# dhansmair/flamingo-mini

Measured on AMD Instinct MI355X. Metric: images/sec (fwd+bwd) flamingo-mini bs=32, higher is better.
Workload: dtype bf16

## Files before the change

flamingo-mini_amd/csrc/ff_optim.hip:

```cpp
#include <algorithm>
#include <cstdlib>
#include <type_traits>
#include "ff_common.h"
#include "ff_internal.h"

namespace ff {

constexpr int kAdamTensors = 32;
constexpr int kAdamChunk = 256 * 128;

struct AdamTable {
    void* p[kAdamTensors];
    const void* g[kAdamTensors];
    void* m[kAdamTensors];
    void* v[kAdamTensors];
    float* w[kAdamTensors];
    long long n[kAdamTensors];
    int block_start[kAdamTensors + 1];
    int count;
    float lr, beta1, beta2, eps, decay, bc1, bc2_sqrt, grad_scale;
    const float* step_dev;
    const float* lr_dev;
    const float* grad_coef;
};

template <typename T, typename ST, bool MASTER, int VEC, int MODE = 0, bool CLIP = false, typename GT = T>
__global__ __launch_bounds__(256) void adamw_kernel(const AdamTable t) {
    int ti = 0;
#pragma unroll 1
    while (ti + 1 < t.count && (int)blockIdx.x >= t.block_start[ti + 1]) ti++;
    const long long n = t.n[ti];
    const long long base = (long long)((int)blockIdx.x - t.block_start[ti]) * kAdamChunk;
    T* p = (T*)t.p[ti];
    const GT* g = (const GT*)t.g[ti];
    ST* m = (ST*)t.m[ti];
    ST* v = (ST*)t.v[ti];
    float* w = t.w[ti];
    float bc1 = t.bc1, bc2_sqrt = t.bc2_sqrt;
    if (t.step_dev) {
        const float step = *t.step_dev;
        bc1 = 1.f - powf(t.beta1, step);
        bc2_sqrt = sqrtf(1.f - powf(t.beta2, step));
    }
    const float lr = t.lr_dev ? *t.lr_dev : t.lr;
    float clip_scale = 0.f;
    if constexpr (CLIP) clip_scale = t.grad_scale * *t.grad_coef;
    const float step_size = lr / bc1, keep = 1.f - lr * t.decay;
    bool vec = VEC > 1 && n % VEC == 0 && ((uintptr_t)p | (uintptr_t)g | (uintptr_t)m | (uintptr_t)v) % 16 == 0;
    if (MASTER) vec = vec && (uintptr_t)w % 16 == 0;
    auto ldv = [&](auto* q, long long i, float (&o)[VEC], auto stream) {
        typedef std::remove_cv_t<std::remove_pointer_t<decltype(q)>> Q;
        constexpr int QN = Vec<Q>::N;
#pragma unroll
        for (int c = 0; c < VEC / QN; c++) {
            float part[QN];
            if constexpr (decltype(stream)::value && MODE >= 1) Vec<Q>::load_nt(q + i + c * QN, part);
            else Vec<Q>::load(q + i + c * QN, part);
#pragma unroll
            for (int e = 0; e < QN; e++) o[c * QN + e] = part[e];
        }
    };
    auto stv = [&](auto* q, long long i, const float (&o)[VEC], auto stream) {
        typedef std::remove_pointer_t<decltype(q)> Q;
        constexpr int QN = Vec<Q>::N;
#pragma unroll
        for (int c = 0; c < VEC / QN; c++) {
            float part[QN];
#pragma unroll
            for (int e = 0; e < QN; e++) part[e] = o[c * QN + e];
            if constexpr (decltype(stream)::value && MODE >= 1) Vec<Q>::store_nt(q + i + c * QN, part);
            else Vec<Q>::store(q + i + c * QN, part);
        }
    };
    const long long end = min(n, base + (long long)kAdamChunk);
    auto update = [&](float (&pf)[VEC], const float (&gf)[VEC], float (&mf)[VEC], float (&vf)[VEC]) {
#pragma unroll
        for (int e = 0; e < VEC; e++) {
            float gr;
            if constexpr (CLIP) gr = gf[e] * clip_scale;
            else gr = gf[e] * t.grad_scale;
            pf[e] *= keep;
            mf[e] = t.beta1 * mf[e] + (1.f - t.beta1) * gr;
            vf[e] = t.beta2 * vf[e] + (1.f - t.beta2) * gr * gr;
            pf[e] -= step_size * mf[e] / (sqrtf(vf[e]) / bc2_sqrt + t.eps);
        }
    };
    if (vec) {
        constexpr std::true_type S{};
        constexpr std::false_type K{};
        auto store = [&](long long i, const float (&pf)[VEC], const float (&mf)[VEC], const float (&vf)[VEC]) {
            stv(p, i, pf, K); stv(m, i, mf, S); stv(v, i, vf, S);
            if (MASTER) stv(w, i, pf, S);
        };
        long long i = base + (long long)threadIdx.x * VEC;
        for (; i + 256 * VEC < end; i += 512 * VEC) {
            const long long j = i + 256 * VEC;
            float p0[VEC], g0[VEC], m0[VEC], v0[VEC], p1[VEC], g1[VEC], m1[VEC], v1[VEC];
            if (MASTER) { ldv(w, i, p0, S); ldv(w, j, p1, S); } else { ldv(p, i, p0, K); ldv(p, j, p1, K); }
            ldv(g, i, g0, S); ldv(g, j, g1, S);
            ldv(m, i, m0, S); ldv(m, j, m1, S);
            ldv(v, i, v0, S); ldv(v, j, v1, S);
            update(p0, g0, m0, v0);
            update(p1, g1, m1, v1);
            store(i, p0, m0, v0);
            store(j, p1, m1, v1);
        }
        if (i < end) {
            float pf[VEC], gf[VEC], mf[VEC], vf[VEC];
            if (MASTER) ldv(w, i, pf, S); else ldv(p, i, pf, K);
            ldv(g, i, gf, S); ldv(m, i, mf, S); ldv(v, i, vf, S);
            update(pf, gf, mf, vf);
            store(i, pf, mf, vf);
        }
        return;
    }
    for (long long i = base + (long long)threadIdx.x * VEC; i < end; i += 256 * VEC) {
        float pf[VEC], gf[VEC], mf[VEC], vf[VEC];
#pragma unroll
        for (int e = 0; e < VEC; e++) {
            const bool ok = i + e < n;
            pf[e] = ok ? (MASTER ? w[i + e] : to_f32(p[i + e])) : 0.f; gf[e] = ok ? to_f32(g[i + e]) : 0.f;
            mf[e] = ok ? to_f32(m[i + e]) : 0.f; vf[e] = ok ? to_f32(v[i + e]) : 0.f;
        }
        update(pf, gf, mf, vf);
#pragma unroll
        for (int e = 0; e < VEC; e++)
            if (i + e < n) {
                p[i + e] = from_f32<T>(pf[e]); m[i + e] = from_f32<ST>(mf[e]); v[i + e] = from_f32<ST>(vf[e]);
                if (MASTER) w[i + e] = pf[e];
            }
    }
}

template <bool CLIP>
static void adamw_dispatch(int dtype, bool master, int state_dtype, dim3 grid, hipStream_t stream, const AdamTable& t) {
    const dim3 block(256);
    if (dtype == FF_DTYPE_F32) adamw_kernel<float, float, false, 4, 0, CLIP><<<grid, block, 0, stream>>>(t);
    else if (master) adamw_kernel<bf16, float, true, 8, 1, CLIP><<<grid, block, 0, stream>>>(t);
    else if (state_dtype == FF_DTYPE_F32) adamw_kernel<bf16, float, false, 8, 1, CLIP><<<grid, block, 0, stream>>>(t);
    else {
        static const int mode = CLIP ? 1 : dbg_switch("FF_ADAMW_MODE", 1);
        if (mode >= 1) adamw_kernel<bf16, bf16, false, 8, 1, CLIP><<<grid, block, 0, stream>>>(t);
        else if constexpr (!CLIP) adamw_kernel<bf16, bf16, false, 8><<<grid, block, 0, stream>>>(t);
    }
}

template <bool CLIP>
static void adamw_dispatch_acc(bool master, int state_dtype, dim3 grid, hipStream_t stream, const AdamTable& t) {
    const dim3 block(256);
    if (master) adamw_kernel<bf16, float, true, 8, 1, CLIP, float><<<grid, block, 0, stream>>>(t);
    else if (state_dtype == FF_DTYPE_F32) adamw_kernel<bf16, float, false, 8, 1, CLIP, float><<<grid, block, 0, stream>>>(t);
    else adamw_kernel<bf16, bf16, false, 8, 1, CLIP, float><<<grid, block, 0, stream>>>(t);
}

static int adamw_launch(const ff_adamw_desc* d, int state_dtype, void* const* params, const void* const* grads, void* const* exp_avg,
                        void* const* exp_avg_sq, float* const* master, const float* lr_dev, const float* grad_coef, const long long* numels,
                        hipStream_t stream, bool acc_grads = false) {
    FF_CHECK(d && params && grads && exp_avg && exp_avg_sq && numels, FF_ERR_SHAPE, "ff_adamw_step: null argument");
    FF_CHECK(d->dtype == FF_DTYPE_F32 || d->dtype == FF_DTYPE_BF16, FF_ERR_UNSUPPORTED, "ff_adamw_step: dtype %d", d->dtype);
    FF_CHECK(state_dtype == d->dtype || state_dtype == FF_DTYPE_F32, FF_ERR_UNSUPPORTED, "ff_adamw_step: moments must be stored in the parameter dtype or in fp32");
    FF_CHECK(!master || d->dtype == FF_DTYPE_BF16, FF_ERR_UNSUPPORTED, "ff_adamw_step: fp32 master copies go with bf16 parameters");
    FF_CHECK(d->n_tensors >= 0 && (d->step >= 1 || d->step_dev), FF_ERR_SHAPE, "ff_adamw_step: n_tensors=%d step=%d", d->n_tensors, d->step);
    AdamTable t;
    t.lr = d->lr; t.beta1 = d->beta1; t.beta2 = d->beta2; t.eps = d->eps; t.decay = d->weight_decay;
    t.step_dev = d->step_dev;
    t.lr_dev = lr_dev;
    t.grad_coef = grad_coef;
    t.bc1 = 1.f - powf(d->beta1, (float)std::max(d->step, 1));
    t.bc2_sqrt = sqrtf(1.f - powf(d->beta2, (float)std::max(d->step, 1)));
    t.grad_scale = d->grad_scale == 0.f ? 1.f : d->grad_scale;
    int i = 0;
    while (i < d->n_tensors) {
        int cnt = 0, blocks = 0;
        while (i < d->n_tensors && cnt < kAdamTensors) {
            if (numels[i] > 0) {
                FF_CHECK(params[i] && grads[i] && exp_avg[i] && exp_avg_sq[i] && (!master || master[i]), FF_ERR_SHAPE, "ff_adamw_step: tensor %d has a null pointer", i);
                t.p[cnt] = params[i]; t.g[cnt] = grads[i]; t.m[cnt] = exp_avg[i]; t.v[cnt] = exp_avg_sq[i]; t.n[cnt] = numels[i];
                t.w[cnt] = master ? master[i] : nullptr;
                t.block_start[cnt] = blocks;
                blocks += cdiv(numels[i], kAdamChunk);
                cnt++;
            }
            i++;
        }
        if (!cnt) break;
        t.block_start[cnt] = blocks;
        t.count = cnt;
        const dim3 grid(blocks);
        if (master) FF_CHECK(state_dtype == FF_DTYPE_F32, FF_ERR_UNSUPPORTED, "ff_adamw_step: fp32 master copies go with fp32 moments");
        if (acc_grads && d->dtype == FF_DTYPE_BF16) {
            if (grad_coef) adamw_dispatch_acc<true>(master != nullptr, state_dtype, grid, stream, t);
            else adamw_dispatch_acc<false>(master != nullptr, state_dtype, grid, stream, t);
        } else if (grad_coef) adamw_dispatch<true>(d->dtype, master != nullptr, state_dtype, grid, stream, t);
        else adamw_dispatch<false>(d->dtype, master != nullptr, state_dtype, grid, stream, t);
        FF_TRY(check_launch("adamw"));
    }
    return FF_OK;
}


struct GradTable {
    void* g[kAdamTensors];
    long long n[kAdamTensors];
    int block_start[kAdamTensors + 1];
    int count;
    float scale;
    float* partials;
    const float* coef;
};
constexpr long long kGradMaxBlocks = 1 << 22;

template <typename T>
__global__ __launch_bounds__(256) void grad_sumsq_kernel(const GradTable t) {
    __shared__ float red[4];
    constexpr int VEC = Vec<T>::N, PIECES = 8;
    int ti = 0;
#pragma unroll 1
    while (ti + 1 < t.count && (int)blockIdx.x >= t.block_start[ti + 1]) ti++;
    const long long n = t.n[ti];
    const long long base = (long long)((int)blockIdx.x - t.block_start[ti]) * kAdamChunk;
    const long long end = min(n, base + (long long)kAdamChunk);
    const T* g = (const T*)t.g[ti];
    const float scale = t.scale;
    float acc = 0.f;
    long long tail = base;
    if ((uintptr_t)g % 16 == 0) {
        const long long vend = base + (end - base) / VEC * VEC;
        tail = vend;
        long long i = base + (long long)threadIdx.x * VEC;
        for (; i + (PIECES - 1) * 256 * VEC < vend; i += PIECES * 256 * VEC) {
            typename Vec<T>::raw r[PIECES];
#pragma unroll
            for (int k = 0; k < PIECES; k++) r[k] = __builtin_nontemporal_load((const typename Vec<T>::raw*)(g + i + k * 256 * VEC));
#pragma unroll
            for (int k = 0; k < PIECES; k++)
#pragma unroll
                for (int e = 0; e < VEC; e++) {
                    const float x = (float)r[k][e] * scale;
                    acc = fmaf(x, x, acc);
                }
        }
        for (; i < vend; i += 256 * VEC) {
            float x[VEC];
            Vec<T>::load_nt(g + i, x);
#pragma unroll
            for (int e = 0; e < VEC; e++) {
                const float y = x[e] * scale;
                acc = fmaf(y, y, acc);
            }
        }
    }
    for (long long i = tail + threadIdx.x; i < end; i += 256) {
        const float x = to_f32(g[i]) * scale;
        acc = fmaf(x, x, acc);
    }
    acc = block_sum<4>(acc, red);
    if (threadIdx.x == 0) t.partials[blockIdx.x] = acc;
}

__global__ __launch_bounds__(1024) void grad_sumsq_reduce_kernel(const float* partials, long long n, double* sum, int accumulate) {
    __shared__ double red[16];
    double s = 0.0;
    long long i = threadIdx.x;
    for (; i + 3 * 1024 < n; i += 4 * 1024) {
        const float a = partials[i], b = partials[i + 1024], c = partials[i + 2048], d = partials[i + 3072];
        s += (double)a; s += (double)b; s += (double)c; s += (double)d;
    }
    for (; i < n; i += 1024) s += (double)partials[i];
#pragma unroll
    for (int o = 32; o > 0; o >>= 1) s += __shfl_xor(s, o, 64);
    if ((threadIdx.x & 63) == 0) red[threadIdx.x >> 6] = s;
    __syncthreads();
    if (threadIdx.x == 0) {
        double total = accumulate ? *sum : 0.0;
        for (int w = 0; w < 16; w++) total += red[w];
        *sum = total;
    }
}

__global__ void grad_clip_coef_kernel(const double* sum, float max_norm, float* norm, float* coef) {
    if (threadIdx.x != 0) return;
    const float nrm = (float)sqrt(*sum);
    const float c = max_norm / (nrm + 1e-6f);
    if (norm) *norm = nrm;
    if (coef) *coef = c > 1.f ? 1.f : c;
}

template <typename T>
__global__ __launch_bounds__(256) void grad_scale_kernel(const GradTable t) {
    constexpr int VEC = Vec<T>::N;
    int ti = 0;
#pragma unroll 1
    while (ti + 1 < t.count && (int)blockIdx.x >= t.block_start[ti + 1]) ti++;
    const long long n = t.n[ti];
    const long long base = (long long)((int)blockIdx.x - t.block_start[ti]) * kAdamChunk;
    const long long end = min(n, base + (long long)kAdamChunk);
    T* g = (T*)t.g[ti];
    const float c = *t.coef;
    long long tail = base;
    if ((uintptr_t)g % 16 == 0) {
        const long long vend = base + (end - base) / VEC * VEC;
        tail = vend;
        for (long long i = base + (long long)threadIdx.x * VEC; i < vend; i += 256 * VEC) {
            float x[VEC];
            Vec<T>::load(g + i, x);
#pragma unroll
            for (int e = 0; e < VEC; e++) x[e] *= c;
            Vec<T>::store(g + i, x);
        }
    }
    for (long long i = tail + threadIdx.x; i < end; i += 256) g[i] = from_f32<T>(to_f32(g[i]) * c);
}

struct AccTable {
    const void* g[kAdamTensors];
    float* a[kAdamTensors];
    long long n[kAdamTensors];
    int block_start[kAdamTensors + 1];
    int count;
    float scale;
};

template <typename T, bool OVERWRITE>
__global__ __launch_bounds__(256) void grad_accumulate_kernel(const AccTable t) {
    constexpr int VEC = Vec<T>::N, PIECES = 4;
    int ti = 0;
#pragma unroll 1
    while (ti + 1 < t.count && (int)blockIdx.x >= t.block_start[ti + 1]) ti++;
    const long long n = t.n[ti];
    const long long base = (long long)((int)blockIdx.x - t.block_start[ti]) * kAdamChunk;
    const long long end = min(n, base + (long long)kAdamChunk);
    const T* g = (const T*)t.g[ti];
    float* a = t.a[ti];
    const float s = t.scale;
    auto lda = [&](long long i, float (&o)[VEC]) {
#pragma unroll
        for (int c = 0; c < VEC / 4; c++) {
            float part[4];
            Vec<float>::load_nt(a + i + c * 4, part);
#pragma unroll
            for (int e = 0; e < 4; e++) o[c * 4 + e] = part[e];
        }
    };
    auto sta = [&](long long i, const float (&o)[VEC]) {
#pragma unroll
        for (int c = 0; c < VEC / 4; c++) {
            float part[4];
#pragma unroll
            for (int e = 0; e < 4; e++) part[e] = o[c * 4 + e];
            Vec<float>::store_nt(a + i + c * 4, part);
        }
    };
    auto fold = [&](float gf, float af) { return OVERWRITE ? s * gf : fmaf(s, gf, af); };
    long long tail = base;
    if (((uintptr_t)g | (uintptr_t)a) % 16 == 0) {
        const long long vend = base + (end - base) / VEC * VEC;
        tail = vend;
        long long i = base + (long long)threadIdx.x * VEC;
        for (; i + (PIECES - 1) * 256 * VEC < vend; i += PIECES * 256 * VEC) {
            float gf[PIECES][VEC], af[PIECES][VEC];
#pragma unroll
            for (int k = 0; k < PIECES; k++) Vec<T>::load_nt(g + i + k * 256 * VEC, gf[k]);
            if constexpr (!OVERWRITE) {
#pragma unroll
                for (int k = 0; k < PIECES; k++) lda(i + k * 256 * VEC, af[k]);
            }
#pragma unroll
            for (int k = 0; k < PIECES; k++) {
#pragma unroll
                for (int e = 0; e < VEC; e++) af[k][e] = fold(gf[k][e], OVERWRITE ? 0.f : af[k][e]);
                sta(i + k * 256 * VEC, af[k]);
            }
        }
        for (; i < vend; i += 256 * VEC) {
            float gf[VEC], af[VEC];
            Vec<T>::load_nt(g + i, gf);
            if constexpr (!OVERWRITE) lda(i, af);
#pragma unroll
            for (int e = 0; e < VEC; e++) af[e] = fold(gf[e], OVERWRITE ? 0.f : af[e]);
            sta(i, af);
        }
    }
    for (long long i = tail + threadIdx.x; i < end; i += 256)
        a[i] = fold(to_f32(g[i]), OVERWRITE ? 0.f : a[i]);
}

static long long grad_slots(int n_tensors, const long long* numels) {
    long long slots = 0;
    for (int i = 0; i < n_tensors; i++)
        if (numels[i] > 0) slots += (numels[i] + kAdamChunk - 1) / kAdamChunk;
    return slots;
}

template <typename F>
static int grad_launches(const char* what, int n_tensors, void* const* grads, const long long* numels, GradTable& t, F&& launch) {
    FF_CHECK(n_tensors >= 0 && (n_tensors == 0 || (grads && numels)), FF_ERR_SHAPE, "%s: null argument", what);
    long long slot = 0;
    int i = 0;
    while (i < n_tensors) {
        int cnt = 0;
        long long blocks = 0;
        while (i < n_tensors && cnt < kAdamTensors) {
            if (numels[i] > 0) {
                const long long b = (numels[i] + kAdamChunk - 1) / kAdamChunk;
                FF_CHECK(b <= kGradMaxBlocks, FF_ERR_SHAPE, "%s: tensor %d has %lld elements", what, i, numels[i]);
                if (blocks + b > kGradMaxBlocks) break;
                FF_CHECK(grads[i], FF_ERR_SHAPE, "%s: tensor %d has a null pointer", what, i);
                t.g[cnt] = grads[i]; t.n[cnt] = numels[i];
                t.block_start[cnt] = (int)blocks;
                blocks += b;
                cnt++;
            }
            i++;
        }
        if (!cnt) break;
        t.block_start[cnt] = (int)blocks;
        t.count = cnt;
        launch(t, (int)blocks, slot);
        FF_TRY(check_launch(what));
        slot += blocks;
    }
    return FF_OK;
}

}

extern "C" int ff_adamw_step(const ff_adamw_desc* d, void* const* params, const void* const* grads, void* const* exp_avg,
                             void* const* exp_avg_sq, const long long* numels, ff_stream_t stream) {
    return ff::adamw_launch(d, d ? d->dtype : 0, params, grads, exp_avg, exp_avg_sq, nullptr, nullptr, nullptr, numels, (hipStream_t)stream);
}
extern "C" int ff_adamw_step_mixed(const ff_adamw_desc* d, int state_dtype, void* const* params, const void* const* grads, void* const* exp_avg,
                                   void* const* exp_avg_sq, float* const* master, const float* lr_dev, const long long* numels,
                                   ff_stream_t stream) {
    return ff::adamw_launch(d, state_dtype, params, grads, exp_avg, exp_avg_sq, master, lr_dev, nullptr, numels, (hipStream_t)stream);
}

extern "C" int ff_adamw_step_clipped(const ff_adamw_desc* d, int state_dtype, void* const* params, const void* const* grads, void* const* exp_avg,
                                     void* const* exp_avg_sq, float* const* master, const float* lr_dev, const float* grad_coef,
                                     const long long* numels, ff_stream_t stream) {
    FF_CHECK(grad_coef, FF_ERR_SHAPE, "ff_adamw_step_clipped: grad_coef is null");
    return ff::adamw_launch(d, state_dtype, params, grads, exp_avg, exp_avg_sq, master, lr_dev, grad_coef, numels, (hipStream_t)stream);
}
extern "C" int ff_adamw_step_acc(const ff_adamw_desc* d, int state_dtype, void* const* params, const float* const* grads32, void* const* exp_avg,
                                 void* const* exp_avg_sq, float* const* master, const float* lr_dev, const float* grad_coef,
                                 const long long* numels, ff_stream_t stream) {
    return ff::adamw_launch(d, state_dtype, params, (const void* const*)grads32, exp_avg, exp_avg_sq, master, lr_dev, grad_coef, numels,
                            (hipStream_t)stream, true);
}
extern "C" long long ff_grad_sumsq_partials(int n_tensors, const long long* numels) {
    return n_tensors > 0 && numels ? ff::grad_slots(n_tensors, numels) : 0;
}
extern "C" int ff_grad_sumsq(int dtype, int n_tensors, const void* const* grads, const long long* numels, float scale, float* partials,
                             long long n_partials, ff_stream_t stream) {
    using namespace ff;
    FF_CHECK(dtype == FF_DTYPE_F32 || dtype == FF_DTYPE_BF16, FF_ERR_UNSUPPORTED, "ff_grad_sumsq: dtype %d", dtype);
    FF_CHECK(n_tensors >= 0 && (n_tensors == 0 || numels), FF_ERR_SHAPE, "ff_grad_sumsq: null argument");
    const long long need = n_tensors > 0 ? grad_slots(n_tensors, numels) : 0;
    FF_CHECK(need <= n_partials && (need == 0 || partials), FF_ERR_WORKSPACE, "ff_grad_sumsq: %lld partials needed, %lld given", need, n_partials);
    GradTable t;
    t.scale = scale;
    t.coef = nullptr;
    return grad_launches("ff_grad_sumsq", n_tensors, (void* const*)grads, numels, t, [&](GradTable& tt, int blocks, long long slot) {
        tt.partials = partials + slot;
        if (dtype == FF_DTYPE_F32) grad_sumsq_kernel<float><<<blocks, 256, 0, (hipStream_t)stream>>>(tt);
        else grad_sumsq_kernel<bf16><<<blocks, 256, 0, (hipStream_t)stream>>>(tt);
    });
}
extern "C" int ff_grad_sumsq_reduce(const float* partials, long long n_partials, double* sum, int accumulate, ff_stream_t stream) {
    FF_CHECK(sum && n_partials >= 0 && (n_partials == 0 || partials), FF_ERR_SHAPE, "ff_grad_sumsq_reduce: null argument");
    ff::grad_sumsq_reduce_kernel<<<1, 1024, 0, (hipStream_t)stream>>>(partials, n_partials, sum, accumulate);
    return ff::check_launch("ff_grad_sumsq_reduce");
}
extern "C" int ff_grad_clip_coef(const double* sum, float max_norm, float* norm, float* coef, ff_stream_t stream) {
    FF_CHECK(sum && (norm || coef), FF_ERR_SHAPE, "ff_grad_clip_coef: null argument");
    ff::grad_clip_coef_kernel<<<1, 64, 0, (hipStream_t)stream>>>(sum, max_norm, norm, coef);
    return ff::check_launch("ff_grad_clip_coef");
}
extern "C" int ff_scale_grads(int dtype, int n_tensors, void* const* grads, const long long* numels, const float* coef, ff_stream_t stream) {
    using namespace ff;
    FF_CHECK(dtype == FF_DTYPE_F32 || dtype == FF_DTYPE_BF16, FF_ERR_UNSUPPORTED, "ff_scale_grads: dtype %d", dtype);
    FF_CHECK(coef, FF_ERR_SHAPE, "ff_scale_grads: coef is null");
    GradTable t;
    t.scale = 1.f;
    t.partials = nullptr;
    t.coef = coef;
    return grad_launches("ff_scale_grads", n_tensors, grads, numels, t, [&](GradTable& tt, int blocks, long long) {
        if (dtype == FF_DTYPE_F32) grad_scale_kernel<float><<<blocks, 256, 0, (hipStream_t)stream>>>(tt);
        else grad_scale_kernel<bf16><<<blocks, 256, 0, (hipStream_t)stream>>>(tt);
    });
}
extern "C" int ff_grad_accumulate(int dtype, int n_tensors, const void* const* grads, float* const* acc, const long long* numels, float scale,
                                  int overwrite, ff_stream_t stream) {
    using namespace ff;
    const char* what = "ff_grad_accumulate";
    FF_CHECK(dtype == FF_DTYPE_F32 || dtype == FF_DTYPE_BF16, FF_ERR_UNSUPPORTED, "%s: dtype %d", what, dtype);
    FF_CHECK(n_tensors >= 0 && (n_tensors == 0 || (grads && acc && numels)), FF_ERR_SHAPE, "%s: null argument", what);
    AccTable t;
    t.scale = scale;
    int i = 0;
    while (i < n_tensors) {
        int cnt = 0;
        long long blocks = 0;
        while (i < n_tensors && cnt < kAdamTensors) {
            if (numels[i] > 0) {
                const long long b = (numels[i] + kAdamChunk - 1) / kAdamChunk;
                FF_CHECK(b <= kGradMaxBlocks, FF_ERR_SHAPE, "%s: tensor %d has %lld elements", what, i, numels[i]);
                if (blocks + b > kGradMaxBlocks) break;
                FF_CHECK(grads[i] && acc[i], FF_ERR_SHAPE, "%s: tensor %d has a null pointer", what, i);
                t.g[cnt] = grads[i]; t.a[cnt] = acc[i]; t.n[cnt] = numels[i];
                t.block_start[cnt] = (int)blocks;
                blocks += b;
                cnt++;
            }
            i++;
        }
        if (!cnt) break;
        t.block_start[cnt] = (int)blocks;
        t.count = cnt;
        const dim3 grid((unsigned)blocks);
        hipStream_t s = (hipStream_t)stream;
        if (dtype == FF_DTYPE_F32) {
            if (overwrite) grad_accumulate_kernel<float, true><<<grid, 256, 0, s>>>(t);
            else grad_accumulate_kernel<float, false><<<grid, 256, 0, s>>>(t);
        } else {
            if (overwrite) grad_accumulate_kernel<bf16, true><<<grid, 256, 0, s>>>(t);
            else grad_accumulate_kernel<bf16, false><<<grid, 256, 0, s>>>(t);
        }
        FF_TRY(check_launch(what));
    }
    return FF_OK;
}
```

Before: 790.4.

## Make AdamW kernel persistent with occupancy-sized grid and smaller work items

The AdamW kernel now runs as a persistent grid-stride loop over smaller work items instead of one block per large chunk. Grid size comes from a cached CU count times the kernel's measured occupancy. Per-block setup (bias correction, lr load) is hoisted out of the item loop, and launch bounds add a minimum-waves hint per dtype. This aims to balance load across tensors of uneven size and cut tail effects, at the cost of a serial tensor-index walk per block and possible register pressure from the occupancy hint.

```diff
diff --git a/flamingo-mini_amd/csrc/ff_optim.hip b/flamingo-mini_amd/csrc/ff_optim.hip
--- a/flamingo-mini_amd/csrc/ff_optim.hip
+++ b/flamingo-mini_amd/csrc/ff_optim.hip
@@ -1,4 +1,5 @@
 #include <algorithm>
+#include <atomic>
 #include <cstdlib>
 #include <type_traits>
 #include "ff_common.h"
@@ -8,6 +9,8 @@
 
 constexpr int kAdamTensors = 32;
 constexpr int kAdamChunk = 256 * 128;
+constexpr int kAdamItem = 256 * 16;
+constexpr long long kAdamMaxItems = 1 << 30;
 
 struct AdamTable {
     void* p[kAdamTensors];
@@ -16,7 +19,7 @@
     void* v[kAdamTensors];
     float* w[kAdamTensors];
     long long n[kAdamTensors];
-    int block_start[kAdamTensors + 1];
+    int item_start[kAdamTensors + 1];
     int count;
     float lr, beta1, beta2, eps, decay, bc1, bc2_sqrt, grad_scale;
     const float* step_dev;
@@ -24,28 +27,14 @@
     const float* grad_coef;
 };
 
-template <typename T, typename ST, bool MASTER, int VEC, int MODE = 0, bool CLIP = false, typename GT = T>
-__global__ __launch_bounds__(256) void adamw_kernel(const AdamTable t) {
-    int ti = 0;
-#pragma unroll 1
-    while (ti + 1 < t.count && (int)blockIdx.x >= t.block_start[ti + 1]) ti++;
+template <typename T, typename ST, bool MASTER, int VEC, int MODE, bool CLIP, typename GT>
+FF_DEV void adamw_item(const AdamTable& t, int ti, long long base, float step_size, float keep, float bc2_sqrt, float clip_scale) {
     const long long n = t.n[ti];
-    const long long base = (long long)((int)blockIdx.x - t.block_start[ti]) * kAdamChunk;
     T* p = (T*)t.p[ti];
     const GT* g = (const GT*)t.g[ti];
     ST* m = (ST*)t.m[ti];
     ST* v = (ST*)t.v[ti];
     float* w = t.w[ti];
-    float bc1 = t.bc1, bc2_sqrt = t.bc2_sqrt;
-    if (t.step_dev) {
-        const float step = *t.step_dev;
-        bc1 = 1.f - powf(t.beta1, step);
-        bc2_sqrt = sqrtf(1.f - powf(t.beta2, step));
-    }
-    const float lr = t.lr_dev ? *t.lr_dev : t.lr;
-    float clip_scale = 0.f;
-    if constexpr (CLIP) clip_scale = t.grad_scale * *t.grad_coef;
-    const float step_size = lr / bc1, keep = 1.f - lr * t.decay;
     bool vec = VEC > 1 && n % VEC == 0 && ((uintptr_t)p | (uintptr_t)g | (uintptr_t)m | (uintptr_t)v) % 16 == 0;
     if (MASTER) vec = vec && (uintptr_t)w % 16 == 0;
     auto ldv = [&](auto* q, long long i, float (&o)[VEC], auto stream) {
@@ -72,7 +61,7 @@
             else Vec<Q>::store(q + i + c * QN, part);
         }
     };
-    const long long end = min(n, base + (long long)kAdamChunk);
+    const long long end = min(n, base + (long long)kAdamItem);
     auto update = [&](float (&pf)[VEC], const float (&gf)[VEC], float (&mf)[VEC], float (&vf)[VEC]) {
 #pragma unroll
         for (int e = 0; e < VEC; e++) {
@@ -132,25 +121,73 @@
     }
 }
 
+template <typename T, typename ST> constexpr int kAdamWaves = std::is_same<T, float>::value ? 6 : std::is_same<ST, float>::value ? 4 : 5;
+
+template <typename T, typename ST, bool MASTER, int VEC, int MODE = 0, bool CLIP = false, typename GT = T>
+__global__ __launch_bounds__(256, (kAdamWaves<T, ST>)) void adamw_kernel(const AdamTable t) {
+    float bc1 = t.bc1, bc2_sqrt = t.bc2_sqrt;
+    if (t.step_dev) {
+        const float step = *t.step_dev;
+        bc1 = 1.f - powf(t.beta1, step);
+        bc2_sqrt = sqrtf(1.f - powf(t.beta2, step));
+    }
+    const float lr = t.lr_dev ? *t.lr_dev : t.lr;
+    float clip_scale = 0.f;
+    if constexpr (CLIP) clip_scale = t.grad_scale * *t.grad_coef;
+    const float step_size = lr / bc1, keep = 1.f - lr * t.decay;
+    const int items = t.item_start[t.count];
+    int ti = 0;
+#pragma unroll 1
+    for (int item = blockIdx.x; item < items; item += gridDim.x) {
+        while (item >= t.item_start[ti + 1]) ti++;
+        adamw_item<T, ST, MASTER, VEC, MODE, CLIP, GT>(t, ti, (long long)(item - t.item_start[ti]) * kAdamItem, step_size, keep, bc2_sqrt, clip_scale);
+    }
+}
+
+template <auto Kernel>
+static int resident_slots() {
+    static std::atomic<int> cache[64];
+    int dev = 0;
+    if (hipGetDevice(&dev) != hipSuccess || dev < 0) return 0;
+    int slots = dev < 64 ? cache[dev].load(std::memory_order_relaxed) : 0;
+    if (slots == 0) {
+        int cus = 0, per_cu = 0;
+        if (hipDeviceGetAttribute(&cus, hipDeviceAttributeMultiprocessorCount, dev) != hipSuccess ||
+            hipOccupancyMaxActiveBlocksPerMultiprocessor(&per_cu, (const void*)Kernel, 256, 0) != hipSuccess || cus <= 0 || per_cu <= 0) {
+            (void)hipGetLastError();
+            return 0;
+        }
+        slots = cus * per_cu;
+        if (dev < 64) cache[dev].store(slots, std::memory_order_relaxed);
+    }
+    return slots;
+}
+
+template <auto Kernel>
+static int adamw_run(hipStream_t stream, const AdamTable& t) {
+    const int slots = resident_slots<Kernel>();
+    FF_CHECK(slots > 0, FF_ERR_LAUNCH, "ff_adamw_step: the device's CU count / the kernel's occupancy could not be queried");
+    Kernel<<<dim3(std::min(t.item_start[t.count], slots)), dim3(256), 0, stream>>>(t);
+    return check_launch("adamw");
+}
+
 template <bool CLIP>
-static void adamw_dispatch(int dtype, bool master, int state_dtype, dim3 grid, hipStream_t stream, const AdamTable& t) {
-    const dim3 block(256);
-    if (dtype == FF_DTYPE_F32) adamw_kernel<float, float, false, 4, 0, CLIP><<<grid, block, 0, stream>>>(t);
-    else if (master) adamw_kernel<bf16, float, true, 8, 1, CLIP><<<grid, block, 0, stream>>>(t);
-    else if (state_dtype == FF_DTYPE_F32) adamw_kernel<bf16, float, false, 8, 1, CLIP><<<grid, block, 0, stream>>>(t);
-    else {
-        static const int mode = CLIP ? 1 : dbg_switch("FF_ADAMW_MODE", 1);
-        if (mode >= 1) adamw_kernel<bf16, bf16, false, 8, 1, CLIP><<<grid, block, 0, stream>>>(t);
-        else if constexpr (!CLIP) adamw_kernel<bf16, bf16, false, 8><<<grid, block, 0, stream>>>(t);
-    }
+static int adamw_dispatch(int dtype, bool master, int state_dtype, hipStream_t stream, const AdamTable& t) {
+    if (dtype == FF_DTYPE_F32) return adamw_run<adamw_kernel<float, float, false, 4, 0, CLIP>>(stream, t);
+    if (master) return adamw_run<adamw_kernel<bf16, float, true, 8, 1, CLIP>>(stream, t);
+    if (state_dtype == FF_DTYPE_F32) return adamw_run<adamw_kernel<bf16, float, false, 8, 1, CLIP>>(stream, t);
+    if constexpr (!CLIP) {
+        static const int mode = dbg_switch("FF_ADAMW_MODE", 1);
+        if (mode < 1) return adamw_run<adamw_kernel<bf16, bf16, false, 8>>(stream, t);
+    }
+    return adamw_run<adamw_kernel<bf16, bf16, false, 8, 1, CLIP>>(stream, t);
 }
 
 template <bool CLIP>
-static void adamw_dispatch_acc(bool master, int state_dtype, dim3 grid, hipStream_t stream, const AdamTable& t) {
-    const dim3 block(256);
-    if (master) adamw_kernel<bf16, float, true, 8, 1, CLIP, float><<<grid, block, 0, stream>>>(t);
-    else if (state_dtype == FF_DTYPE_F32) adamw_kernel<bf16, float, false, 8, 1, CLIP, float><<<grid, block, 0, stream>>>(t);
-    else adamw_kernel<bf16, bf16, false, 8, 1, CLIP, float><<<grid, block, 0, stream>>>(t);
+static int adamw_dispatch_acc(bool master, int state_dtype, hipStream_t stream, const AdamTable& t) {
+    if (master) return adamw_run<adamw_kernel<bf16, float, true, 8, 1, CLIP, float>>(stream, t);
+    if (state_dtype == FF_DTYPE_F32) return adamw_run<adamw_kernel<bf16, float, false, 8, 1, CLIP, float>>(stream, t);
+    return adamw_run<adamw_kernel<bf16, bf16, false, 8, 1, CLIP, float>>(stream, t);
 }
 
 static int adamw_launch(const ff_adamw_desc* d, int state_dtype, void* const* params, const void* const* grads, void* const* exp_avg,
@@ -171,29 +208,31 @@
     t.grad_scale = d->grad_scale == 0.f ? 1.f : d->grad_scale;
     int i = 0;
     while (i < d->n_tensors) {
-        int cnt = 0, blocks = 0;
+        int cnt = 0;
+        long long items = 0;
         while (i < d->n_tensors && cnt < kAdamTensors) {
             if (numels[i] > 0) {
+                const long long k = (numels[i] + kAdamItem - 1) / kAdamItem;
+                FF_CHECK(k <= kAdamMaxItems, FF_ERR_SHAPE, "ff_adamw_step: tensor %d has %lld elements", i, numels[i]);
+                if (items + k > kAdamMaxItems) break;
                 FF_CHECK(params[i] && grads[i] && exp_avg[i] && exp_avg_sq[i] && (!master || master[i]), FF_ERR_SHAPE, "ff_adamw_step: tensor %d has a null pointer", i);
                 t.p[cnt] = params[i]; t.g[cnt] = grads[i]; t.m[cnt] = exp_avg[i]; t.v[cnt] = exp_avg_sq[i]; t.n[cnt] = numels[i];
                 t.w[cnt] = master ? master[i] : nullptr;
-                t.block_start[cnt] = blocks;
-                blocks += cdiv(numels[i], kAdamChunk);
+                t.item_start[cnt] = (int)items;
+                items += k;
                 cnt++;
             }
             i++;
         }
         if (!cnt) break;
-        t.block_start[cnt] = blocks;
+        t.item_start[cnt] = (int)items;
         t.count = cnt;
-        const dim3 grid(blocks);
         if (master) FF_CHECK(state_dtype == FF_DTYPE_F32, FF_ERR_UNSUPPORTED, "ff_adamw_step: fp32 master copies go with fp32 moments");
         if (acc_grads && d->dtype == FF_DTYPE_BF16) {
-            if (grad_coef) adamw_dispatch_acc<true>(master != nullptr, state_dtype, grid, stream, t);
-            else adamw_dispatch_acc<false>(master != nullptr, state_dtype, grid, stream, t);
-        } else if (grad_coef) adamw_dispatch<true>(d->dtype, master != nullptr, state_dtype, grid, stream, t);
-        else adamw_dispatch<false>(d->dtype, master != nullptr, state_dtype, grid, stream, t);
-        FF_TRY(check_launch("adamw"));
+            if (grad_coef) FF_TRY(adamw_dispatch_acc<true>(master != nullptr, state_dtype, stream, t));
+            else FF_TRY(adamw_dispatch_acc<false>(master != nullptr, state_dtype, stream, t));
+        } else if (grad_coef) FF_TRY(adamw_dispatch<true>(d->dtype, master != nullptr, state_dtype, stream, t));
+        else FF_TRY(adamw_dispatch<false>(d->dtype, master != nullptr, state_dtype, stream, t));
     }
     return FF_OK;
 }
```

Result: no change. 790.3 (-0.0%).
